# etri/bwa-mem-scale

Hardware: AMD Instinct MI355X
Metric: Mreads/sec through the GPU hot path (seed -> chain -> extend -> dedup, reads and index resident), 150bp SE vs a synthetic genome of GRCh38 size, at 1 MI355X; % HBM roofline in roofline.frac (higher is better)
Workload: dtype int64 intervals / int16 DP (two columns per register; int32 for queries beyond 191 bases or scores beyond 2^14)

## Files before the change

bwa-mem-scale_amd/csrc/api_extend.hip:

```cpp
#include <cstddef>

#include "stage_state.h"

using namespace bwams;

extern "C" {
static int ext_args(bwams_batch *b, StageState *s, const bwams_mem_opt_t *opt, ExtArgs *A) {
    const int64_t n1 = s->ch.nseq + 1;
    A->chains = s->ch.chains.p; A->n_chains = s->ch.n_chains; A->seeds = s->ch.seeds.p; A->n_seeds = s->ch.n_seeds;
    A->chain_off = s->ch.chain_off.as<int64_t>(); A->seed_off = s->ch.chain_off.as<int64_t>() + n1; A->enc = b->d_enc.p; A->cum = b->d_cum.p;
    A->nseq = s->ch.nseq; A->ref = b->idx->fmi.ref;
    int rc = dev_bns(b->idx, &A->bns);
    if (rc) return rc;
    A->opt = *opt; A->regs = s->ext.regs.p; A->srt = s->ext.srt.p; A->rmax = s->ext.rmax.as<int64_t>(); A->cnt = s->ext.cnt.as<int32_t>();
    A->ctr = b->d_ctr.p; A->state = s->ext.state.p; A->kreg = s->ext.kreg.p; A->cur = s->ext.cur.p; A->lim = s->ext.lim.p; A->sel_heavy = s->heavy.p;
    A->n_sel_heavy = &b->d_ctr.p->sel_heavy; A->sel_ticket = b->d_ctr.p->ext_sel_ticket; A->req_list = s->ext.req_list.p; A->rtask = nullptr;
    return BWAMS_OK;
}

static hipError_t ext_round_clear(bwams_batch *b) {
    DevCounters *c = b->d_ctr.p;
    return hipMemsetAsync(&c->ext_n_req, 0, (size_t)((char *)(c->ext_n_retry + 2) - (char *)&c->ext_n_req), b->stream);
}
static int ext_round_fetch(bwams_batch *b, int64_t *n_req, int64_t *n_rest, int64_t *n_l, int64_t *n_r) {
    DevCounters *h = b->h_ctr.p;
    BWAMS_HIP(hipMemcpyAsync(&h->ext_n_req, &b->d_ctr.p->ext_n_req, 3 * sizeof(unsigned long long), hipMemcpyDeviceToHost, b->stream));
    BWAMS_HIP(hipStreamSynchronize(b->stream));
    *n_req = (int64_t)h->ext_n_req; *n_rest = (int64_t)h->ext_n_rest;
    *n_l = (int64_t)(h->ext_n_tasks & 0xffffffffull); *n_r = (int64_t)(h->ext_n_tasks >> 32);
    return BWAMS_OK;
}

static int ext_plan(bwams_batch *b, StageState *s, const bwams_mem_opt_t *opt, int extend_all, ExtArgs *A) {
    const int64_t N1 = s->ch.n_seeds + 1, n1 = s->ch.nseq + 1;
    BWAMS_HIP(s->ext.regs.ensure_n((size_t)N1)); BWAMS_HIP(s->ext.srt.ensure_n((size_t)N1));
    BWAMS_HIP(s->ext.rmax.ensure((size_t)(s->ch.n_chains + 1) * 16)); BWAMS_HIP(s->ext.cnt.ensure((size_t)N1 * 6 * 4));
    BWAMS_HIP(s->ext.state.ensure_n((size_t)N1)); BWAMS_HIP(s->ext.kreg.ensure((size_t)N1 * 32)); BWAMS_HIP(s->ext.cur.ensure_n((size_t)n1));
    BWAMS_HIP(s->ext.lim.ensure_n((size_t)n1)); BWAMS_HIP(s->heavy.ensure_n((size_t)n1));
    BWAMS_HIP(s->ext.req_list.ensure_n((size_t)N1)); BWAMS_HIP(s->ext.rtask.ensure_n((size_t)N1));
    int rc = ext_args(b, s, opt, A);
    if (rc) return rc;
    BWAMS_HIP(hipMemsetAsync(&b->d_ctr.p->sel_heavy, 0, sizeof(unsigned long long), b->stream));
    BWAMS_HIP(ext_round_clear(b));
    launch_ext_heavy_list(*A, b->stream);
    BWAMS_HIP(hipMemsetAsync(s->ext.cur.p, 0, (size_t)n1 * 4, b->stream));
    BWAMS_HIP(hipMemsetAsync(s->ext.lim.p, 0, (size_t)n1 * 4, b->stream));
    launch_ext_plan(*A, extend_all, b->stream);
    return BWAMS_OK;
}

static int ext_build_flat(bwams_batch *b, StageState *s, const ExtArgs &A, const int32_t *list, int64_t n, int64_t tot[6]) {
    hipStream_t st = b->stream;
    const int64_t n1 = n + 1;
    BWAMS_HIP(s->ext.ewide.ensure((size_t)n1 * 6 * 8)); BWAMS_HIP(s->ext.eoffs.ensure((size_t)n1 * 6 * 8));
    launch_ext_widen(A, list, n, s->ext.ewide.as<int64_t>(), st);
    int rc = scan_rows(b, s->ext.ewide.as<int64_t>(), s->ext.eoffs.as<int64_t>(), 6, n1);
    if (rc) return rc;
    for (int r = 0; r < 6; ++r) BWAMS_HIP(hipMemcpyAsync(&tot[r], s->ext.eoffs.as<int64_t>() + r * n1 + n, 8, hipMemcpyDeviceToHost, st));
    BWAMS_HIP(hipStreamSynchronize(st));
    for (int r : {1, 2, 4, 5})
        if (tot[r] >= ((int64_t)1 << 31)) {
            set_last_error("extension task buffers exceed the 31-bit offsets of SeqPair; use smaller chunks");
            return BWAMS_ERR_CAPACITY;
        }
    s->ext.n_left = tot[0]; s->ext.lqer_b = tot[1]; s->ext.lref_b = tot[2];
    s->ext.n_right = tot[3]; s->ext.rqer_b = tot[4]; s->ext.rref_b = tot[5];
    BWAMS_HIP(s->ext.lpairs.ensure_n((size_t)(tot[0] + 1))); BWAMS_HIP(s->ext.rpairs.ensure_n((size_t)(tot[3] + 1)));
    const int64_t mx = tot[0] > tot[3] ? tot[0] : tot[3];
    BWAMS_HIP(s->ext.retry.ensure_n((size_t)(mx + 1)));
    s->ext.tasks_inplace = false;
    BWAMS_HIP(s->ext.lqer.ensure_n((size_t)tot[1] + 64)); BWAMS_HIP(s->ext.lref.ensure_n((size_t)tot[2] + 64));
    BWAMS_HIP(s->ext.rqer.ensure_n((size_t)tot[4] + 64)); BWAMS_HIP(s->ext.rref.ensure_n((size_t)tot[5] + 64));
    if (tot[0] + tot[3] > 0)
        launch_ext_build(A, list, n, s->ext.eoffs.as<int64_t>(), s->ext.lpairs.p, s->ext.lref.p, s->ext.lqer.p, s->ext.rpairs.p, s->ext.rref.p,
                         s->ext.rqer.p, nullptr, nullptr, st);
    return BWAMS_OK;
}

static int ext_build_round(bwams_batch *b, StageState *s, const ExtArgs &A, int64_t n_req, int64_t n_l, int64_t n_r, bool inplace) {
    if (!inplace) {
        int64_t tot[6] = {0, 0, 0, 0, 0, 0};
        if (int rc = ext_build_flat(b, s, A, A.req_list, n_req, tot)) return rc;
        if (tot[0] != n_l || tot[3] != n_r) {
            set_last_error("bwams_extend_run: the request list and its task counters disagree");
            return BWAMS_ERR_DEVICE;
        }
        return BWAMS_OK;
    }
    s->ext.n_left = n_l; s->ext.n_right = n_r;
    s->ext.lqer_b = s->ext.lref_b = s->ext.rqer_b = s->ext.rref_b = 0;
    BWAMS_HIP(s->ext.lpairs.ensure_n((size_t)(n_l + 1))); BWAMS_HIP(s->ext.rpairs.ensure_n((size_t)(n_r + 1)));
    const int64_t mx = n_l > n_r ? n_l : n_r;
    BWAMS_HIP(s->ext.retry.ensure_n((size_t)(mx + 1)));
    s->ext.tasks_inplace = true;
    BWAMS_HIP(s->ext.lsrc.ensure((size_t)(n_l + 1) * 16)); BWAMS_HIP(s->ext.rsrc.ensure((size_t)(n_r + 1) * 16));
    if (n_l + n_r > 0) launch_ext_build(A, A.req_list, n_req, nullptr, s->ext.lpairs.p, nullptr, nullptr, s->ext.rpairs.p,
                         nullptr, nullptr, s->ext.lsrc.as<int64_t>(), s->ext.rsrc.as<int64_t>(), b->stream);
    return BWAMS_OK;
}

int bwams_extend_build(bwams_batch_t *b, const bwams_mem_opt_t *opt, int64_t *n_left, int64_t *n_right) {
    if (!b || !b->stages || !b->stages->ch.done) {
        set_last_error("bwams_extend_build: run bwams_chain_run (or bwams_chain_upload) first");
        return BWAMS_ERR_ARG;
    }
    if (!b->idx->fmi.ref) {
        set_last_error("bwams_extend_build: the index was opened without its .0123 reference");
        return BWAMS_ERR_ARG;
    }
    int rc = check_opt(opt, "bwams_extend_build");
    if (rc) return rc;
    BWAMS_HIP(hipSetDevice(b->idx->device));
    StageState *s = b->stages;
    outdated(s, From::built);
    hipStream_t st = b->stream;
    ExtArgs A;
    BWAMS_HIP(hipEventRecord(s->ev[2], st));
    if ((rc = ext_plan(b, s, opt, 1, &A))) return rc;
    int64_t tot[6];
    if ((rc = ext_build_flat(b, s, A, nullptr, s->ch.n_seeds, tot))) return rc;
    BWAMS_HIP(hipEventRecord(s->ev[3], st));
    BWAMS_HIP(hipGetLastError());
    s->ext.built = true;
    s->opt = *opt;
    if (n_left) *n_left = tot[0];
    if (n_right) *n_right = tot[3];
    return BWAMS_OK;
}

static int run_side(bwams_batch *b, StageState *s, const ExtArgs &A, int right, int64_t *n_retry_out) {
    hipStream_t st = b->stream;
    bwams_seqpair_t *pairs = right ? s->ext.rpairs.p : s->ext.lpairs.p;
    const bool ip = s->ext.tasks_inplace;
    const uint8_t *ref = ip ? A.ref : (right ? s->ext.rref.p : s->ext.lref.p);
    const uint8_t *qer = ip ? A.enc : (right ? s->ext.rqer.p : s->ext.lqer.p);
    const int64_t *src = ip ? (right ? s->ext.rsrc.as<int64_t>() : s->ext.lsrc.as<int64_t>()) : nullptr;
    const int dir = ip && !right ? -1 : 1;
    const int64_t n = right ? s->ext.n_right : s->ext.n_left;
    SwParams prm;
    sw_params(A.opt, right ? A.opt.pen_clip3 : A.opt.pen_clip5, &prm);
    const int qmax = b->max_read_len > 1 ? b->max_read_len : 1;
    if (n == 0) return BWAMS_OK;
    unsigned long long *d_nretry = &b->d_ctr.p->ext_n_retry[right], *h_nretry = &b->h_ctr.p->ext_n_retry[right];
    bwams_seqpair_t *rp = A.rtask ? s->ext.rpairs.p : nullptr;
    if (bsw_list_bytes(n) > b->sw.d_bsw_list.cap) BWAMS_HIP(hipStreamSynchronize(st));
    BWAMS_HIP(b->sw.d_bsw_list.ensure(bsw_list_bytes(n), bsw_list_bytes(n + n / 4 + 1024)));
    if (int lrc = launch_bsw(pairs, n, ref, qer, A.opt.w, prm, qmax, b->d_ctr.p, b->cu_count, st, b->sw.d_bsw_list.p, s->aux, s->fork, s->join, src, dir)) {
        set_last_error(lrc == -2 ? "banded SW: a query longer than ~18000 bases does not fit the LDS kernel" : "banded SW: stream fork/join failed");
        return lrc == -2 ? BWAMS_ERR_UNSUPPORTED : BWAMS_ERR_DEVICE;
    }
    launch_ext_post(A, right, pairs, n, A.opt.w, 0, s->ext.retry.p, d_nretry, rp, st);
    BWAMS_HIP(hipMemcpyAsync(h_nretry, d_nretry, sizeof(unsigned long long), hipMemcpyDeviceToHost, st));
    BWAMS_HIP(hipStreamSynchronize(st));
    const unsigned long long nr = *h_nretry;
    if (nr) {
        if (launch_bsw(s->ext.retry.p, (int64_t)nr, ref, qer, A.opt.w << 1, prm, qmax, b->d_ctr.p, b->cu_count, st, b->sw.d_bsw_list.p, s->aux, s->fork, s->join, src, dir)) return BWAMS_ERR_DEVICE;
        launch_ext_post(A, right, s->ext.retry.p, (int64_t)nr, A.opt.w << 1, 1, nullptr, d_nretry, rp, st);
    }
    *n_retry_out += (int64_t)nr;
    return BWAMS_OK;
}

int bwams_extend_run(bwams_batch_t *b, const bwams_mem_opt_t *opt, int64_t *n_regs) {
    if (!b || !b->stages || !b->stages->ch.done) {
        set_last_error("bwams_extend_run: run bwams_chain_run (or bwams_chain_upload) first");
        return BWAMS_ERR_ARG;
    }
    if (!b->idx->fmi.ref) {
        set_last_error("bwams_extend_run: the index was opened without its .0123 reference");
        return BWAMS_ERR_ARG;
    }
    int rc = check_opt(opt, "bwams_extend_run");
    if (rc) return rc;
    int kMaxRounds = 6;
    if (knobs().ext_max_rounds > 0) kMaxRounds = knobs().ext_max_rounds;
    const bool adaptive_off = knobs().ext_all_rounds != 0;
    const bool inplace_on = knobs().ext_inplace != 0;
    StageState *s = b->stages;
    BWAMS_HIP(hipSetDevice(b->idx->device));
    hipStream_t st = b->stream;
    outdated(s, From::built);
    ExtArgs A;
    BWAMS_HIP(hipEventRecord(s->ev[10], st));
    BWAMS_HIP(hipMemsetAsync(&b->d_ctr.p->bsw_cells, 0, sizeof(unsigned long long), st));
    BWAMS_HIP(hipEventRecord(s->ev[2], st));
    if ((rc = ext_plan(b, s, opt, opt->extend_all != 0, &A))) return rc;
    A.rtask = s->ext.rtask.p;
    int64_t tot_left = 0, tot_right = 0;
    s->ext.n_retry_left = s->ext.n_retry_right = 0;
    int64_t n_req = 0, n_rest = 0, n_l = 0, n_r = 0;
    if ((rc = ext_round_fetch(b, &n_req, &n_rest, &n_l, &n_r))) return rc;
    int round = 0;
    for (;; ++round) {
        if ((rc = ext_build_round(b, s, A, n_req, n_l, n_r, inplace_on))) return rc;
        if (round == 0) { BWAMS_HIP(hipEventRecord(s->ev[3], st)); BWAMS_HIP(hipEventRecord(s->ev[4], st)); }
        tot_left += n_l; tot_right += n_r;
        if ((rc = run_side(b, s, A, 0, &s->ext.n_retry_left))) return rc;
        if (round == 0) { BWAMS_HIP(hipEventRecord(s->ev[5], st)); BWAMS_HIP(hipEventRecord(s->ev[6], st)); }
        if ((rc = run_side(b, s, A, 1, &s->ext.n_retry_right))) return rc;
        if (round == 0) { BWAMS_HIP(hipEventRecord(s->ev[7], st)); BWAMS_HIP(hipEventRecord(s->ev[8], st)); }
        BWAMS_HIP(ext_round_clear(b));
        const bool verbose_sel = knobs().verbose != 0;
        if (verbose_sel) BWAMS_HIP(hipMemsetAsync(b->d_ctr.p->dbg, 0, sizeof b->d_ctr.p->dbg, st));
        if (s->ch.n_seeds && launch_ext_select(A, b->cu_count, st, s->aux, s->fork, s->join)) {
            set_last_error("bwams_extend_run: stream fork/join failed");
            return BWAMS_ERR_DEVICE;
        }
        if (verbose_sel) {
            unsigned long long d[16];
            BWAMS_HIP(hipMemcpyAsync(d, b->d_ctr.p->dbg, sizeof d, hipMemcpyDeviceToHost, st));
            BWAMS_HIP(hipStreamSynchronize(st));
            if (d[0])
                fprintf(stderr, "[bwams_extend_run] selection walk, round %d: %llu reads, Mticks total %.2f fetch %.2f bulk scan %.2f ordered part %.2f (of it keep-anyway %.2f); "
                                "%llu slots, %llu keep-anyway calls; longest read: %.3f Mticks (fetch %.3f bulk %.3f ordered %.3f, of it keep-anyway %.3f), %llu slots "
                                "%llu calls, %llu kept regions\n",
                        round, d[0], d[1] / 1e6, d[2] / 1e6, d[3] / 1e6, d[4] / 1e6, d[5] / 1e6, d[6], d[7], d[8] / 1e6, d[9] / 1e6, d[10] / 1e6, d[11] / 1e6,
                        d[12] / 1e6, d[13], d[14], d[15]);
        }
        if (round == 0) BWAMS_HIP(hipEventRecord(s->ev[9], st));
        if ((rc = ext_round_fetch(b, &n_req, &n_rest, &n_l, &n_r))) return rc;
        if (n_req == 0) break;
        const bool few_left = !adaptive_off && (n_req + n_rest) * 32 < tot_left + tot_right;
        if (round + 1 >= kMaxRounds || few_left) {
            launch_ext_request_rest(A, st);
            if ((rc = ext_round_fetch(b, &n_req, &n_rest, &n_l, &n_r))) return rc;
        }
    }
    BWAMS_HIP(hipEventRecord(s->ev[11], st));
    BWAMS_HIP(hipGetLastError());
    s->ext.n_rounds = round + 1;
    s->ext.n_left = tot_left; s->ext.n_right = tot_right;
    s->ext.done = true;
    s->opt = *opt;
    if (n_regs) *n_regs = s->ch.n_seeds;
    return BWAMS_OK;
}

int bwams_extend_fetch(bwams_batch_t *b, bwams_alnreg_t *regs, int64_t reg_cap, int64_t *reg_off, int32_t *seed_aln) {
    if (!b || !b->stages || !(b->stages->ext.done || b->stages->ext.built)) {
        set_last_error("bwams_extend_fetch: no regions on the device");
        return BWAMS_ERR_ARG;
    }
    StageState *s = b->stages;
    if (s->ch.n_seeds > reg_cap) return BWAMS_ERR_CAPACITY;
    BWAMS_HIP(hipSetDevice(b->idx->device));
    hipStream_t st = b->stream;
    if (s->ch.n_seeds) BWAMS_HIP(hipMemcpyAsync(regs, s->ext.regs.p, (size_t)s->ch.n_seeds * sizeof(bwams_alnreg_t), hipMemcpyDeviceToHost, st));
    if (reg_off) BWAMS_HIP(hipMemcpyAsync(reg_off, s->ch.chain_off.as<int64_t>() + (s->ch.nseq + 1), (size_t)(s->ch.nseq + 1) * 8, hipMemcpyDeviceToHost, st));
    if (seed_aln && s->ch.n_seeds)
        BWAMS_HIP(hipMemcpy2DAsync(seed_aln, 4, reinterpret_cast<const char *>(s->ch.seeds.p) + offsetof(bwams_chain_seed_t, aln),
                                   sizeof(bwams_chain_seed_t), 4, (size_t)s->ch.n_seeds, hipMemcpyDeviceToHost, st));
    BWAMS_HIP(hipStreamSynchronize(st));
    return BWAMS_OK;
}

int bwams_extend_tasks_fetch(bwams_batch_t *b, int32_t side, bwams_seqpair_t *pairs, int64_t pair_cap, uint8_t *ref,
                             int64_t ref_cap, uint8_t *qer, int64_t qer_cap, int64_t *n_pairs, int64_t *ref_bytes,
                             int64_t *qer_bytes) {
    if (!b || !b->stages || !(b->stages->ext.built || b->stages->ext.done) || (side != 0 && side != 1)) {
        set_last_error("bwams_extend_tasks_fetch: no task lists on the device");
        return BWAMS_ERR_ARG;
    }
    if (b->stages->ext.tasks_inplace) {
        set_last_error("bwams_extend_tasks_fetch: bwams_extend_run extends in place and builds no flat task buffers; bwams_extend_build does");
        return BWAMS_ERR_ARG;
    }
    StageState *s = b->stages;
    const int64_t n = side ? s->ext.n_right : s->ext.n_left, rb = side ? s->ext.rref_b : s->ext.lref_b, qb = side ? s->ext.rqer_b : s->ext.lqer_b;
    if (n_pairs) *n_pairs = n;
    if (ref_bytes) *ref_bytes = rb;
    if (qer_bytes) *qer_bytes = qb;
    if (n > pair_cap || rb > ref_cap || qb > qer_cap) return BWAMS_ERR_CAPACITY;
    BWAMS_HIP(hipSetDevice(b->idx->device));
    hipStream_t st = b->stream;
    if (n) BWAMS_HIP(hipMemcpyAsync(pairs, side ? s->ext.rpairs.p : s->ext.lpairs.p, (size_t)n * sizeof(bwams_seqpair_t), hipMemcpyDeviceToHost, st));
    if (rb) BWAMS_HIP(hipMemcpyAsync(ref, side ? s->ext.rref.p : s->ext.lref.p, (size_t)rb, hipMemcpyDeviceToHost, st));
    if (qb) BWAMS_HIP(hipMemcpyAsync(qer, side ? s->ext.rqer.p : s->ext.lqer.p, (size_t)qb, hipMemcpyDeviceToHost, st));
    BWAMS_HIP(hipStreamSynchronize(st));
    return BWAMS_OK;
}
}
```

bwa-mem-scale_amd/csrc/bsw_extend.hip:

```cpp
#include "common.h"
#include "wave_ops.h"

namespace bwams {

namespace {

constexpr int kWavesPerBlock = 4;
constexpr int kTaskChunk = 8;
constexpr size_t kBswLdsMax = 160 * 1024;

__host__ __device__ __forceinline__ size_t bsw_row_bytes(int qmax) {
    return (((size_t)(qmax + 1) * 8 + (size_t)qmax + 64 + 15) / 16) * 16;
}

__device__ __forceinline__ int wave_incl_prefix_max(int v, int lane) {
#pragma unroll
    for (int o = 1; o < 64; o <<= 1) {
        const int t = __shfl_up(v, o);
        if (lane >= o) v = max(v, t);
    }
    return v;
}

__global__ __launch_bounds__(kWavesPerBlock * 64) void bsw_kernel(
// ... 390 lines not shown
                const int e = Ev[c];
                int h = Mv[c] > e ? Mv[c] : e;
                h = h > F ? h : F;
                int e2 = Mv[c] - oe_del;
                e2 = e2 > 0 ? e2 : 0;
                const int e1 = e - e_del;
                e2 = e2 > e1 ? e2 : e1;
                Hh[c] = h; E2[c] = e2;
            }
            const int h_in = grp_shr1<LPT>(Hh[kWin - 1], c_h, g);
#pragma unroll
            for (int c = 0; c < kWin; ++c) {
                const int j = jb + c;
                const bool act = in && j < end;
                const int hl = c ? Hh[c - 1] : h_in;
                if (act) {
                    const uint32_t he = (uint32_t)hl | ((uint32_t)E2[c] << 14);
                    row_eh[j] = (he & 0x0fffffffu) | (Qb[c] & ~0x0fffffffu);
                    const int k = (Hh[c] << 8) | j;
                    key = key > k ? key : k;
                    if (hl != 0 || E2[c] != 0) { first_nz = first_nz < j ? first_nz : j; last_nz = j; }
                }
            }
            {
                const int cl = end - 1 - jb;
                if (in && cl >= 0 && cl < kWin) {
                    int hv = Hh[0];
#pragma unroll
                    for (int c = 1; c < kWin; ++c) hv = cl == c ? Hh[c] : hv;
                    hlast = hv;
                }
            }
            if (wave_any(row && base + LPT * kWin < end)) {
                const int pm = grp_all_max<LPT>(scan);
                c_max = c_max > pm ? c_max : pm;
                c_h = grp_all_max<LPT>(g == LPT - 1 ? Hh[kWin - 1] : -1);
            }
        }
        key = grp_all_max<LPT>(key);
        first_nz = -grp_all_max<LPT>(-first_nz);
        last_nz = grp_all_max<LPT>(last_nz);
        hlast = grp_all_max<LPT>(hlast);
        const int m = row ? key >> 8 : 0, mj = row ? key & 0xff : -1;
        const int h1f = row ? hlast : h1;
        if (alive) {
            if (g == 0) {
                row_eh[end] = (uint32_t)h1f | (row_eh[end] & 0xf0000000u);
            }
            if (row) cells += (unsigned long long)(g == 0 ? end - beg : 0);
            const int j_exit = row ? end : beg;
            if (j_exit == qlen) {
                max_ie = gscore > h1f ? max_ie : i;
                gscore = gscore > h1f ? gscore : h1f;
            }
            bool fin = m == 0;
            if (!fin) {
                if (m > mx) {
                    mx = m; max_i = i; max_j = mj;
                    int d = mj - i;
                    d = d < 0 ? -d : d;
                    max_off = max_off > d ? max_off : d;
                } else if (prm.zdrop > 0) {
                    if (i - max_i > mj - max_j) fin = mx - m - ((i - max_i) - (mj - max_j)) * e_del > prm.zdrop;
                    else fin = mx - m - ((mj - max_j) - (i - max_i)) * e_ins > prm.zdrop;
                }
            }
            if (!fin) {
                const int nbeg = first_nz < end ? first_nz : end;
                int jj;
                if (h1f != 0) jj = end;
                else if (last_nz >= nbeg) jj = last_nz;
                else jj = nbeg - 1;
                beg = nbeg;
                end = jj + 2 < qlen ? jj + 2 : qlen;
                ++i;
                fin = i >= tlen;
            }
            if (fin) {
                if (g == 0) {
                    bwams_seqpair_t *o = &pairs[cur];
                    o->score = mx; o->qle = max_j + 1; o->tle = max_i + 1; o->gtle = max_ie + 1; o->gscore = gscore; o->max_off = max_off;
                }
                alive = false;
            }
        }
    }
    for (int o = 32; o > 0; o >>= 1) cells += ((unsigned long long)__shfl_down((unsigned)(cells >> 32), o) << 32) | (unsigned)__shfl_down((unsigned)cells, o);
    if (lane == 0 && cells) atomicAdd(&ctr->bsw_cells, cells);
}


namespace pk {
__device__ __forceinline__ uint32_t add(uint32_t a, uint32_t b) { uint32_t d; asm("v_pk_add_u16 %0, %1, %2" : "=v"(d) : "v"(a), "v"(b)); return d; }
__device__ __forceinline__ uint32_t sub(uint32_t a, uint32_t b) { uint32_t d; asm("v_pk_sub_i16 %0, %1, %2" : "=v"(d) : "v"(a), "v"(b)); return d; }
__device__ __forceinline__ uint32_t max(uint32_t a, uint32_t b) { uint32_t d; asm("v_pk_max_i16 %0, %1, %2" : "=v"(d) : "v"(a), "v"(b)); return d; }
__device__ __forceinline__ uint32_t max0(uint32_t a) { uint32_t d; asm("v_pk_max_i16 %0, %1, 0" : "=v"(d) : "v"(a)); return d; }
__device__ __forceinline__ uint32_t minu(uint32_t a, uint32_t b) { uint32_t d; asm("v_pk_min_u16 %0, %1, %2" : "=v"(d) : "v"(a), "v"(b)); return d; }
__device__ __forceinline__ uint32_t mul(uint32_t a, uint32_t b) { uint32_t d; asm("v_pk_mul_lo_u16 %0, %1, %2" : "=v"(d) : "v"(a), "v"(b)); return d; }
__device__ __forceinline__ uint32_t hi2(uint32_t a) { return __builtin_amdgcn_perm(a, a, 0x03020302u); }
__device__ __forceinline__ uint32_t lo2(uint32_t a) { return __builtin_amdgcn_perm(a, a, 0x01000100u); }
__device__ __forceinline__ uint32_t bfi(uint32_t mask, uint32_t a, uint32_t b) { return (a & mask) | (b & ~mask); }
template <int CTRL> __device__ __forceinline__ int qdpp(int v) { return __builtin_amdgcn_update_dpp(0, v, CTRL, 0xF, 0xF, false); }
__device__ __forceinline__ int quad_all_max(int v) {
    int t = qdpp<0xB1>(v);
    v = v > t ? v : t;
    t = qdpp<0x4E>(v);
    return v > t ? v : t;
}
}

constexpr int kPkNeg = -16384;
#ifndef BWAMS_PK_WAVES
#define BWAMS_PK_WAVES 2
#endif
constexpr int kPkWaves = BWAMS_PK_WAVES;

__host__ __device__ __forceinline__ bool bsw_pk_eligible(const SwParams &prm) {
    for (int i = 0; i < 5; ++i)
        if (prm.mat[i * 5 + 4] != -1 || prm.mat[4 * 5 + i] != -1) return false;
    return prm.e_ins >= 0 && prm.e_ins <= 64 && prm.e_del >= 0 && prm.e_del <= 64 && prm.o_ins >= 0 && prm.o_ins + prm.e_ins < 8000 &&
           prm.o_del >= 0 && prm.o_del + prm.e_del < 8000;
}

__global__ __launch_bounds__(kPkWaves * 64) void bsw_pk_kernel(
    bwams_seqpair_t *__restrict__ pairs, const int32_t *__restrict__ list, const unsigned long long *n_list_p,
    const uint8_t *__restrict__ ref, const uint8_t *__restrict__ qer, int w0, SwParams prm, DevCounters *ctr, unsigned long long *head,
    int cols, const int64_t *__restrict__ src, int dir) {
    extern __shared__ __align__(16) uint32_t pk_lds[];
    constexpr int LPT = 4, TPW = 16;
    const int lane = threadIdx.x & 63, g = lane & (LPT - 1), q = lane / LPT;
    const int P = cols >> 1;
    uint32_t *const t_hp = pk_lds + 16 + (size_t)((threadIdx.x >> 6) * TPW + q) * (size_t)((5 * P) / 2 + 6);
    uint32_t *const t_ep = t_hp + P + 2;
    uint16_t *const t_sel = reinterpret_cast<uint16_t *>(t_ep + P + 2);
    uint16_t *const t_hp16 = reinterpret_cast<uint16_t *>(t_hp), *const t_ep16 = reinterpret_cast<uint16_t *>(t_ep);
    const int o_del = prm.o_del, e_del = prm.e_del, o_ins = prm.o_ins, e_ins = prm.e_ins;
    const int oe_del = o_del + e_del, oe_ins = o_ins + e_ins;
    uint2 *const pk_tab16 = reinterpret_cast<uint2 *>(pk_lds);
    if (threadIdx.x < 5) {
        const int t = threadIdx.x;
        pk_tab16[t] = make_uint2((uint32_t)(uint16_t)(int16_t)prm.mat[t * 5 + 0] | ((uint32_t)(uint16_t)(int16_t)prm.mat[t * 5 + 1] << 16),
                                 (uint32_t)(uint16_t)(int16_t)prm.mat[t * 5 + 2] | ((uint32_t)(uint16_t)(int16_t)prm.mat[t * 5 + 3] << 16));
    }
    __syncthreads();
    const uint32_t ONE = 0x00010001u, TWO = 0x00020002u, C257 = 0x01010101u;
    const uint32_t OEI = (uint32_t)oe_ins * 0x10001u, OED = (uint32_t)oe_del * 0x10001u, EDX = (uint32_t)e_del * 0x10001u;
    const uint32_t E1X = (uint32_t)e_ins * 0x10001u, E2X = (uint32_t)(2 * e_ins) * 0x10001u;
    const uint32_t NEGP = (uint32_t)(uint16_t)(int16_t)kPkNeg * 0x10001u;
    const int64_t n_list = (int64_t)*n_list_p;
    const unsigned long long kLeaders = 0x1111111111111111ull;
    int64_t pid = 0, pid_end = 0;
    bool exhausted = false;
    bool alive = false;
    int cur = 0, qlen = 0, tlen = 0, h0 = 0, w = 0, i = 0, beg = 0, end = 0;
    int mx = 0, max_i = -1, max_j = -1, max_ie = -1, gscore = -1, max_off = 0, tb_next = 4;
    const uint8_t *tr = ref;
    unsigned long long cells = 0;
    bool start_row = true, row = false;
    int base = 0, h1 = 0, key = -1, hlast = -1, c_max = kPkNeg, c_h = 0;
    uint32_t nzl = 0u, nzf = 0u;
    uint2 tt = make_uint2(0u, 0u);

    for (;;) {
        const unsigned long long need_m = __ballot(!alive);
        if (need_m) {
            if (pid >= pid_end && !exhausted) {
                pid = (int64_t)wave_ticket(head, (unsigned long long)kQuadChunk);
                pid_end = pid + kQuadChunk < n_list ? pid + kQuadChunk : n_list;
                if (pid >= n_list) { exhausted = true; pid_end = pid; }
            }
            const int avail = (int)(pid_end - pid);
            const int nq = __popcll(need_m & kLeaders);
            const int rank = __popcll(need_m & kLeaders & ((1ull << (q * LPT)) - 1ull));
            if (!alive && rank < avail) {
                cur = list[pid + rank];
                const bwams_seqpair_t sp = pairs[cur];
                qlen = sp.len2; tlen = sp.len1; h0 = sp.h0;
                const uint8_t *tq = qer + (src ? src[2 * (int64_t)sp.id] : (int64_t)sp.idq);
                tr = ref + (src ? src[2 * (int64_t)sp.id + 1] : (int64_t)sp.idr);
                start_row = true;
                for (int p = g; p <= (qlen >> 1); p += LPT) {
                    uint32_t hh = 0, ss = 0;
#pragma unroll
                    for (int k = 0; k < 2; ++k) {
                        const int c = 2 * p + k;
                        int h = 0;
                        if (c <= qlen) { h = h0; if (c >= 1) { h = h0 - oe_ins - (c - 1) * e_ins; h = h > 0 ? h : 0; } }
                        uint32_t qb = c < qlen ? (uint32_t)tq[c * dir] : 4u;
                        const uint32_t sel = qb < 4u ? 2u * qb : 0x0du;
                        hh |= (uint32_t)h << (16 * k);
                        ss |= sel << (8 * k);
                    }
                    t_hp[p] = hh; t_ep[p] = 0u; t_sel[p] = (uint16_t)ss;
                }
                w = w0;
                {
                    int max_ins = (int)((double)(qlen * prm.max_sc + prm.end_bonus - o_ins) / e_ins + 1.);
                    max_ins = max_ins > 1 ? max_ins : 1;
                    w = w < max_ins ? w : max_ins;
                    int max_del = (int)((double)(qlen * prm.max_sc + prm.end_bonus - o_del) / e_del + 1.);
                    max_del = max_del > 1 ? max_del : 1;
                    w = w < max_del ? w : max_del;
                }
                mx = h0; max_i = -1; max_j = -1; max_ie = -1; gscore = -1; max_off = 0;
                beg = 0; end = qlen; i = 0;
                alive = tlen > 0;
                if (!alive && g == 0) {
                    bwams_seqpair_t *o = &pairs[cur];
                    o->score = mx; o->qle = 0; o->tle = 0; o->gtle = 0; o->gscore = -1; o->max_off = 0;
                }
                tb_next = alive ? (int)tr[0] : 4;
            }
            pid += nq < avail ? nq : avail;
            if (exhausted && !wave_any(alive)) break;
        }

        if (alive && start_row) {
            int tb = tb_next;
            tb = tb > 4 ? 4 : tb;
            if (i + 1 < tlen) tb_next = tr[(i + 1) * dir];
            tt = pk_tab16[tb];
            if (beg < i - w) beg = i - w;
            if (end > i + w + 1) end = i + w + 1;
            if (end > qlen) end = qlen;
            h1 = 0;
            if (beg == 0) {
                h1 = h0 - (o_del + e_del * (i + 1));
                h1 = h1 < 0 ? 0 : h1;
            }
            row = beg < end;
            key = -1; hlast = -1; nzl = 0u; nzf = 0u;
            c_max = kPkNeg; c_h = 0;
            base = beg & ~3;
            start_row = false;
        }
        {
            const bool in = alive && row;
            const int jb = base + g * 8;
            const bool inr = in && jb < cols;
            int lo = beg - jb, hi = end - jb;
            lo = lo < 0 ? 0 : (lo > 8 ? 8 : lo);
            hi = hi < 0 ? 0 : (hi > 8 ? 8 : hi);
            const uint32_t m8 = inr ? ((1u << hi) - 1u) & ~((1u << lo) - 1u) : 0u;
            const int pj = inr ? (jb >> 1) : 0;
            const uint2 hpa = *reinterpret_cast<const uint2 *>(t_hp + pj), hpb = *reinterpret_cast<const uint2 *>(t_hp + pj + 2);
            const uint2 epa = *reinterpret_cast<const uint2 *>(t_ep + pj), epb = *reinterpret_cast<const uint2 *>(t_ep + pj + 2);
            uint2 sl2;
            sl2.x = *reinterpret_cast<const uint32_t *>(t_sel + pj);
            sl2.y = *reinterpret_cast<const uint32_t *>(t_sel + pj + 2);
            const uint32_t hpv[4] = {hpa.x, hpa.y, hpb.x, hpb.y}, epv[4] = {epa.x, epa.y, epb.x, epb.y};
            const uint32_t slv[4] = {__builtin_amdgcn_perm(sl2.x, sl2.x, 0x01010000u) + 0x01000100u, __builtin_amdgcn_perm(sl2.x, sl2.x, 0x03030202u) + 0x01000100u,
                                     __builtin_amdgcn_perm(sl2.y, sl2.y, 0x01010000u) + 0x01000100u, __builtin_amdgcn_perm(sl2.y, sl2.y, 0x03030202u) + 0x01000100u};
            uint32_t AM[4], M[4], E[4], PX[4], JE[4], JP[4];
            JE[0] = (uint32_t)(jb * e_ins) * 0x10001u + ((uint32_t)e_ins << 16);
            JP[0] = (uint32_t)jb * 0x10001u + 0x00020001u;
#pragma unroll
            for (int c = 1; c < 4; ++c) { JE[c] = pk::add(JE[c - 1], E2X); JP[c] = pk::add(JP[c - 1], TWO); }
            uint32_t Hm[4], T1[4], T2[4];
#pragma unroll
            for (int c = 0; c < 4; ++c) {
                const uint32_t blo = (uint32_t)__builtin_amdgcn_sbfe((int)m8, 2 * c, 1), bhi = (uint32_t)__builtin_amdgcn_sbfe((int)m8, 2 * c + 1, 1);
                AM[c] = pk::bfi(0xffffu, blo, bhi);
            }
#pragma unroll
            for (int c = 0; c < 4; ++c) { Hm[c] = hpv[c] & AM[c]; E[c] = epv[c] & AM[c]; }
#pragma unroll
            for (int c = 0; c < 4; ++c) T1[c] = pk::add(Hm[c], __builtin_amdgcn_perm(tt.y, tt.x, slv[c]));
#pragma unroll
            for (int c = 0; c < 4; ++c) T2[c] = pk::minu(Hm[c], ONE);
#pragma unroll
            for (int c = 0; c < 4; ++c) M[c] = pk::mul(T1[c], T2[c]);
#pragma unroll
            for (int c = 0; c < 4; ++c) T1[c] = pk::sub(M[c], OEI);
#pragma unroll
            for (int c = 0; c < 4; ++c) T1[c] = pk::max0(T1[c]);
#pragma unroll
            for (int c = 0; c < 4; ++c) T1[c] = pk::add(T1[c], JE[c]);
#pragma unroll
            for (int c = 0; c < 4; ++c) PX[c] = pk::max(T1[c], T1[c] << 16);
#pragma unroll
            for (int c = 1; c < 4; ++c) PX[c] = pk::max(PX[c], pk::hi2(PX[c - 1]));
            int scan = (int)(PX[3] >> 16);
            {
                int t = pk::qdpp<0x90>(scan);
                scan = scan > t ? scan : t;
                t = pk::qdpp<0x44>(scan);
                scan = scan > t ? scan : t;
            }
            int Lex = pk::qdpp<0x90>(scan);
            Lex = g == 0 ? kPkNeg : Lex;
            Lex = Lex > c_max ? Lex : c_max;
            const uint32_t Lexp = pk::lo2((uint32_t)Lex);
            uint32_t Hn[4], E2[4], F4[4], ME[4];
#pragma unroll
            for (int c = 0; c < 4; ++c) F4[c] = __builtin_amdgcn_alignbit(PX[c], c ? PX[c - 1] : NEGP, 16);
#pragma unroll
            for (int c = 0; c < 4; ++c) { F4[c] = pk::max(F4[c], Lexp); E2[c] = pk::sub(M[c], OED); }
#pragma unroll
            for (int c = 0; c < 4; ++c) { F4[c] = pk::sub(F4[c], JE[c]); T1[c] = pk::sub(E[c], EDX); ME[c] = pk::max(M[c], E[c]); }
#pragma unroll
            for (int c = 0; c < 4; ++c) { F4[c] = pk::add(F4[c], E1X); E2[c] = pk::max(E2[c], T1[c]); }
#pragma unroll
            for (int c = 0; c < 4; ++c) { F4[c] = pk::max0(F4[c]); E2[c] = pk::max0(E2[c]); }
#pragma unroll
            for (int c = 0; c < 4; ++c) Hn[c] = pk::max(ME[c], F4[c]);
            const int h3 = (int)(Hn[3] >> 16);
            int hin = pk::qdpp<0x90>(h3);
            hin = g == 0 ? c_h : hin;
            uint32_t HL[4];
            HL[0] = __builtin_amdgcn_alignbit(Hn[0], (uint32_t)hin << 16, 16);
#pragma unroll
            for (int c = 1; c < 4; ++c) HL[c] = __builtin_amdgcn_alignbit(Hn[c], Hn[c - 1], 16);
            if (m8) {
                *reinterpret_cast<uint2 *>(t_hp + pj) = make_uint2(pk::bfi(AM[0], HL[0], hpv[0]), pk::bfi(AM[1], HL[1], hpv[1]));
                *reinterpret_cast<uint2 *>(t_hp + pj + 2) = make_uint2(pk::bfi(AM[2], HL[2], hpv[2]), pk::bfi(AM[3], HL[3], hpv[3]));
                *reinterpret_cast<uint2 *>(t_ep + pj) = make_uint2(pk::bfi(AM[0], E2[0], epv[0]), pk::bfi(AM[1], E2[1], epv[1]));
                *reinterpret_cast<uint2 *>(t_ep + pj + 2) = make_uint2(pk::bfi(AM[2], E2[2], epv[2]), pk::bfi(AM[3], E2[3], epv[3]));
            }
            int lkey = -1;
#pragma unroll
            for (int c = 0; c < 4; ++c) {
                const uint32_t ha = Hn[c] & AM[c];
                const int k0 = (int)__builtin_amdgcn_perm(ha, JP[c], 0x0c050400u), k1 = (int)__builtin_amdgcn_perm(ha, JP[c], 0x0c070602u);
                const int kk = k0 > k1 ? k0 : k1;
                lkey = lkey > kk ? lkey : kk;
            }
            {
                uint32_t NF[4], NA[4], NB[4];
#pragma unroll
                for (int c = 0; c < 4; ++c) NF[c] = (HL[c] | E2[c]) & AM[c];
#pragma unroll
                for (int c = 0; c < 4; ++c) { NF[c] = pk::minu(NF[c], ONE); NB[c] = pk::sub(C257, JP[c]); }
#pragma unroll
                for (int c = 0; c < 4; ++c) { NA[c] = pk::mul(NF[c], JP[c]); NB[c] = pk::mul(NF[c], NB[c]); }
                NA[0] = pk::max(NA[0], NA[1]); NA[2] = pk::max(NA[2], NA[3]); NB[0] = pk::max(NB[0], NB[1]); NB[2] = pk::max(NB[2], NB[3]);
                NA[0] = pk::max(NA[0], NA[2]); NB[0] = pk::max(NB[0], NB[2]);
                nzl = pk::max(nzl, NA[0]);
                nzf = pk::max(nzf, NB[0]);
            }
            lkey = m8 ? lkey : -1;
            key = key > lkey ? key : lkey;
            {
                const int oe = hi - 1;
                if (m8 && jb + hi == end) {
                    uint32_t hv = Hn[0];
                    hv = (oe >> 1) == 1 ? Hn[1] : hv;
                    hv = (oe >> 1) == 2 ? Hn[2] : hv;
                    hv = (oe >> 1) == 3 ? Hn[3] : hv;
                    hlast = (int)((hv >> ((oe & 1) << 4)) & 0xffffu);
                }
            }
            if (in && base == (beg & ~3) && h1 != 0 && g == 0) t_hp16[beg] = (uint16_t)h1;
            const int pm = pk::qdpp<0xFF>(scan);
            const int ch = pk::qdpp<0xFF>(h3);
            const bool more = in && base + LPT * 8 < end;
            if (more) {
                c_max = c_max > pm ? c_max : pm;
                c_h = ch;
                base += LPT * 8;
            }
            const int rkey = pk::quad_all_max(key), rhl = pk::quad_all_max(hlast);
            const int a_ = (int)(nzl & 0xffffu), b_ = (int)(nzl >> 16), c_ = (int)(nzf & 0xffffu), d_ = (int)(nzf >> 16);
            int last_nz = pk::quad_all_max(a_ > b_ ? a_ : b_) - 1;
            int first_nz = 256 - pk::quad_all_max(c_ > d_ ? c_ : d_);
            if (alive && !more) {
                if (row && h1 != 0) {
                    first_nz = first_nz < beg ? first_nz : beg;
                    last_nz = last_nz > beg ? last_nz : beg;
                }
                const int m = row ? rkey >> 8 : 0, mj = row ? (rkey & 0xff) - 1 : -1;
                const int h1f = row ? rhl : h1;
                if (g == 0) { t_hp16[end] = (uint16_t)h1f; t_ep16[end] = 0; }
                if (row) cells += (unsigned long long)(g == 0 ? end - beg : 0);
                const int j_exit = row ? end : beg;
                if (j_exit == qlen) {
                    max_ie = gscore > h1f ? max_ie : i;
                    gscore = gscore > h1f ? gscore : h1f;
                }
                bool fin = m == 0;
                if (!fin) {
                    if (m > mx) {
                        mx = m; max_i = i; max_j = mj;
                        int d = mj - i;
                        d = d < 0 ? -d : d;
                        max_off = max_off > d ? max_off : d;
                    } else if (prm.zdrop > 0) {
                        if (i - max_i > mj - max_j) fin = mx - m - ((i - max_i) - (mj - max_j)) * e_del > prm.zdrop;
                        else fin = mx - m - ((mj - max_j) - (i - max_i)) * e_ins > prm.zdrop;
                    }
                }
                if (!fin) {
                    const int nbeg = first_nz < end ? first_nz : end;
                    int jj;
                    if (h1f != 0) jj = end;
                    else if (last_nz >= nbeg) jj = last_nz;
                    else jj = nbeg - 1;
                    beg = nbeg;
                    end = jj + 2 < qlen ? jj + 2 : qlen;
                    ++i;
                    fin = i >= tlen;
                }
                if (fin) {
                    if (g == 0) {
                        bwams_seqpair_t *o = &pairs[cur];
                        o->score = mx; o->qle = max_j + 1; o->tle = max_i + 1; o->gtle = max_ie + 1; o->gscore = gscore; o->max_off = max_off;
                    }
                    alive = false;
                }
                start_row = true;
            }
        }
    }
    for (int o = 32; o > 0; o >>= 1) cells += ((unsigned long long)__shfl_down((unsigned)(cells >> 32), o) << 32) | (unsigned)__shfl_down((unsigned)cells, o);
    if (lane == 0 && cells) atomicAdd(&ctr->bsw_cells, cells);
}

__global__ void bsw_reset_kernel(DevCounters *ctr) {
    for (int i = 0; i < 4; ++i) ctr->bsw_head[i] = 0;
    for (int i = 0; i < kNumBswClass; ++i) ctr->bsw_cls_cnt[i] = ctr->bsw_cls_head[i] = 0;
}

}

int launch_bsw(bwams_seqpair_t *pairs, int64_t n, const uint8_t *ref, const uint8_t *qer, int w, const SwParams &prm, int qmax,
               DevCounters *ctr, int cu_count, hipStream_t st, int32_t *list, hipStream_t *aux, hipEvent_t fork, hipEvent_t *join,
               const int64_t *src, int dir) {
    bsw_reset_kernel<<<1, 1, 0, st>>>(ctr);
    if (n <= 0) return 0;
    bsw_classify_kernel<<<(unsigned)((n + 1023) / 1024), 1024, 0, st>>>(pairs, n, prm.max_sc, list, ctr->bsw_cls_cnt);
    int64_t blocks = (n + kWavesPerBlock - 1) / kWavesPerBlock;
    const int64_t maxb = (int64_t)cu_count * 8;
    if (blocks > maxb) blocks = maxb;
    hipStream_t q[5] = {st, st, st, st, st};
    const int n_aux = aux ? 4 : 0;
    if (n_aux) {
        if (hipEventRecord(fork, st) != hipSuccess) return -1;
        for (int c = 0; c < n_aux; ++c) {
            q[c + 1] = aux[c];
            if (hipStreamWaitEvent(q[c + 1], fork, 0) != hipSuccess) return -1;
        }
    }
    const unsigned B = (unsigned)blocks, T = kWavesPerBlock * 64;
    unsigned long long *cnt = ctr->bsw_cls_cnt, *hd = ctr->bsw_cls_head;
    auto pk_lds = [](int cols) { return (size_t)64 + (size_t)kPkWaves * 16 * ((size_t)(cols / 2) * 10 + 24); };
    {
        static std::mutex mu;
        static bool done[64] = {};
        int dev = 0;
        if (hipGetDevice(&dev) != hipSuccess) return -1;
        std::lock_guard<std::mutex> g(mu);
        if (dev < 0 || dev >= 64 || !done[dev]) {
            if (hipFuncSetAttribute(reinterpret_cast<const void *>(bsw_qwin_kernel<kBswLpt, kBswWin>), hipFuncAttributeMaxDynamicSharedMemorySize,
                                    (int)((size_t)kWavesPerBlock * (64 / kBswLpt) * 192 * 4)) != hipSuccess) return -1;
            if (hipFuncSetAttribute(reinterpret_cast<const void *>(bsw_pk_kernel), hipFuncAttributeMaxDynamicSharedMemorySize, (int)pk_lds(192)) != hipSuccess) return -1;
            if (dev >= 0 && dev < 64) done[dev] = true;
        }
    }
    const bool pk_env = knobs().bsw_pk != 0;
    if (pk_env && bsw_pk_eligible(prm)) {
        static const int kCols[5] = {32, 64, 96, 144, 192};
        const unsigned Bp = (unsigned)((int64_t)B * kWavesPerBlock / kPkWaves);
        for (int c = 4; c >= 0; --c)
            bsw_pk_kernel<<<Bp, kPkWaves * 64, pk_lds(kCols[c]), q[c]>>>(pairs, list + (int64_t)c * n, cnt + c, ref, qer, w, prm, ctr, hd + c, kCols[c], src, dir);
    } else {
    bsw_qwin_kernel<kBswLpt, kBswWin><<<B, T, (size_t)kWavesPerBlock * (64 / kBswLpt) * 192 * 4, q[4]>>>(pairs, list + 4 * n, cnt + 4, ref, qer, w, prm, ctr, hd + 4, 192, src, dir);
    bsw_qwin_kernel<kBswLpt, kBswWin><<<B, T, (size_t)kWavesPerBlock * (64 / kBswLpt) * 144 * 4, q[3]>>>(pairs, list + 3 * n, cnt + 3, ref, qer, w, prm, ctr, hd + 3, 144, src, dir);
    bsw_qwin_kernel<kBswLpt, kBswWin><<<B, T, (size_t)kWavesPerBlock * (64 / kBswLpt) * 96 * 4, q[2]>>>(pairs, list + 2 * n, cnt + 2, ref, qer, w, prm, ctr, hd + 2, 96, src, dir);
    bsw_qwin_kernel<kBswLpt, kBswWin><<<B, T, (size_t)kWavesPerBlock * (64 / kBswLpt) * 64 * 4, q[1]>>>(pairs, list + 1 * n, cnt + 1, ref, qer, w, prm, ctr, hd + 1, 64, src, dir);
    bsw_qwin_kernel<kBswLpt, kBswWin><<<B, T, (size_t)kWavesPerBlock * (64 / kBswLpt) * 32 * 4, q[0]>>>(pairs, list + 0 * n, cnt + 0, ref, qer, w, prm, ctr, hd + 0, 32, src, dir);
    }
    {
        const int waves = bsw_lds_waves(qmax);
        if (waves < 1) return -2;
        const size_t lds = bsw_row_bytes(qmax) * (size_t)waves;
        if (lds > 48 * 1024)
            (void)hipFuncSetAttribute(reinterpret_cast<const void *>(bsw_kernel),
                                      hipFuncAttributeMaxDynamicSharedMemorySize, (int)lds);
        int64_t lblocks = (n + waves - 1) / waves;
        const int64_t lcap = qmax > 16 * kQuadCpl[4] - 1 ? maxb : (int64_t)cu_count * 2;
        if (lblocks > lcap) lblocks = lcap;
        bsw_kernel<<<(unsigned)lblocks, waves * 64, lds, q[0]>>>(pairs, n, ref, qer, w, prm, qmax, -1, ctr, &ctr->bsw_head[3], list + 5 * n, cnt + 5, src, dir);
    }
    if (n_aux)
        for (int c = 0; c < n_aux; ++c) {
            if (hipEventRecord(join[c], q[c + 1]) != hipSuccess) return -1;
            if (hipStreamWaitEvent(st, join[c], 0) != hipSuccess) return -1;
        }
    return 0;
}
size_t bsw_list_bytes(int64_t n) { return (size_t)kNumBswClass * (size_t)(n > 0 ? n : 1) * sizeof(int32_t); }

int bsw_lds_waves(int qmax) {
    const size_t waves = kBswLdsMax / bsw_row_bytes(qmax);
    return waves < (size_t)kWavesPerBlock ? (int)waves : kWavesPerBlock;
}

}
```

Baseline: 10.01.

## Prefetch task metadata per chunk and cooperatively fill query rows across whole wave

When a wave grabs a chunk of tasks, each of the first kQuadChunk lanes loads one task's pair record, offsets, first ref base and band width, and these are broadcast by shuffle to the lanes that take a task. Query-profile and initial H-row setup is then done by all 64 lanes together, one task at a time, using 4-byte vector loads instead of a per-quad strided loop. The aim is to cut the serialized refill cost in the banded SW packed kernel. It adds shuffles, a per-slot fill loop and LDS fences, plus optional timing instrumentation behind a debug macro and a verbose flag.

```diff
diff --git a/bwa-mem-scale_amd/csrc/api_extend.hip b/bwa-mem-scale_amd/csrc/api_extend.hip
--- a/bwa-mem-scale_amd/csrc/api_extend.hip
+++ b/bwa-mem-scale_amd/csrc/api_extend.hip
@@ -145,6 +145,8 @@
     bwams_seqpair_t *rp = A.rtask ? s->ext.rpairs.p : nullptr;
     if (bsw_list_bytes(n) > b->sw.d_bsw_list.cap) BWAMS_HIP(hipStreamSynchronize(st));
     BWAMS_HIP(b->sw.d_bsw_list.ensure(bsw_list_bytes(n), bsw_list_bytes(n + n / 4 + 1024)));
+    const bool verbose_bsw = knobs().verbose != 0;
+    if (verbose_bsw) BWAMS_HIP(hipMemsetAsync(b->d_ctr.p->dbg + 40, 0, 8 * sizeof(unsigned long long), st));
     if (int lrc = launch_bsw(pairs, n, ref, qer, A.opt.w, prm, qmax, b->d_ctr.p, b->cu_count, st, b->sw.d_bsw_list.p, s->aux, s->fork, s->join, src, dir)) {
         set_last_error(lrc == -2 ? "banded SW: a query longer than ~18000 bases does not fit the LDS kernel" : "banded SW: stream fork/join failed");
         return lrc == -2 ? BWAMS_ERR_UNSUPPORTED : BWAMS_ERR_DEVICE;
@@ -152,6 +154,14 @@
     launch_ext_post(A, right, pairs, n, A.opt.w, 0, s->ext.retry.p, d_nretry, rp, st);
     BWAMS_HIP(hipMemcpyAsync(h_nretry, d_nretry, sizeof(unsigned long long), hipMemcpyDeviceToHost, st));
     BWAMS_HIP(hipStreamSynchronize(st));
+    if (verbose_bsw) {
+        unsigned long long d[8];
+        BWAMS_HIP(hipMemcpy(d, b->d_ctr.p->dbg + 40, sizeof d, hipMemcpyDeviceToHost));
+        if (d[6])
+            fprintf(stderr, "[run_side] bsw_pk_kernel, %s, %lld tasks: %llu waves, Mticks of wave-time %.2f, in the refill branch %.2f (%.1f %%), in the pass %.2f; "
+                            "%llu refill events, %llu slots filled, %llu iterations\n",
+                    right ? "right" : "left", (long long)n, d[6], d[0] / 1e6, d[1] / 1e6, 100. * (double)d[1] / (double)d[0], d[2] / 1e6, d[3], d[4], d[5]);
+    }
     const unsigned long long nr = *h_nretry;
     if (nr) {
         if (launch_bsw(s->ext.retry.p, (int64_t)nr, ref, qer, A.opt.w << 1, prm, qmax, b->d_ctr.p, b->cu_count, st, b->sw.d_bsw_list.p, s->aux, s->fork, s->join, src, dir)) return BWAMS_ERR_DEVICE;
diff --git a/bwa-mem-scale_amd/csrc/bsw_extend.hip b/bwa-mem-scale_amd/csrc/bsw_extend.hip
--- a/bwa-mem-scale_amd/csrc/bsw_extend.hip
+++ b/bwa-mem-scale_amd/csrc/bsw_extend.hip
@@ -566,6 +566,9 @@
     int64_t pid = 0, pid_end = 0;
     bool exhausted = false;
     bool alive = false;
+    int64_t pid0 = 0, s_qo = 0, s_to = 0;
+    int s_cur = 0, s_tlen = 0, s_w = 0;
+    uint32_t s_qh = 0u;
     int cur = 0, qlen = 0, tlen = 0, h0 = 0, w = 0, i = 0, beg = 0, end = 0;
     int mx = 0, max_i = -1, max_j = -1, max_ie = -1, gscore = -1, max_off = 0, tb_next = 4;
     const uint8_t *tr = ref;
@@ -574,60 +577,115 @@
     int base = 0, h1 = 0, key = -1, hlast = -1, c_max = kPkNeg, c_h = 0;
     uint32_t nzl = 0u, nzf = 0u;
     uint2 tt = make_uint2(0u, 0u);
+#ifdef BWAMS_BSWDBG
+    const unsigned long long T0 = __builtin_amdgcn_s_memtime();
+    unsigned long long t_refill = 0, t_pass = 0, n_events = 0, n_filled = 0, n_iter = 0;
+#endif
 
     for (;;) {
         const unsigned long long need_m = __ballot(!alive);
         if (need_m) {
+#ifdef BWAMS_BSWDBG
+            const unsigned long long Ta = __builtin_amdgcn_s_memtime();
+#endif
             if (pid >= pid_end && !exhausted) {
                 pid = (int64_t)wave_ticket(head, (unsigned long long)kQuadChunk);
                 pid_end = pid + kQuadChunk < n_list ? pid + kQuadChunk : n_list;
                 if (pid >= n_list) { exhausted = true; pid_end = pid; }
+                pid0 = pid;
+                if (lane < kQuadChunk && pid + lane < pid_end) {
+                    s_cur = list[pid + lane];
+                    const bwams_seqpair_t *sp = &pairs[s_cur];
+                    const int l2 = sp->len2, hh0 = sp->h0;
+                    s_tlen = sp->len1;
+                    if (src) { const int64_t id = sp->id; s_qo = src[2 * id]; s_to = src[2 * id + 1]; }
+                    else { s_qo = (int64_t)sp->idq; s_to = (int64_t)sp->idr; }
+                    uint32_t tb = s_tlen > 0 ? (uint32_t)ref[s_to] : 4u;
+                    tb = tb > 4u ? 4u : tb;
+                    s_qh = (uint32_t)l2 | ((uint32_t)hh0 << 8) | (tb << 24);
+                    int ww = w0;
+                    int max_ins = (int)((double)(l2 * prm.max_sc + prm.end_bonus - o_ins) / e_ins + 1.);
+                    max_ins = max_ins > 1 ? max_ins : 1;
+                    ww = ww < max_ins ? ww : max_ins;
+                    int max_del = (int)((double)(l2 * prm.max_sc + prm.end_bonus - o_del) / e_del + 1.);
+                    max_del = max_del > 1 ? max_del : 1;
+                    s_w = ww < max_del ? ww : max_del;
+                }
             }
             const int avail = (int)(pid_end - pid);
             const int nq = __popcll(need_m & kLeaders);
             const int rank = __popcll(need_m & kLeaders & ((1ull << (q * LPT)) - 1ull));
-            if (!alive && rank < avail) {
-                cur = list[pid + rank];
-                const bwams_seqpair_t sp = pairs[cur];
-                qlen = sp.len2; tlen = sp.len1; h0 = sp.h0;
-                const uint8_t *tq = qer + (src ? src[2 * (int64_t)sp.id] : (int64_t)sp.idq);
-                tr = ref + (src ? src[2 * (int64_t)sp.id + 1] : (int64_t)sp.idr);
-                start_row = true;
-                for (int p = g; p <= (qlen >> 1); p += LPT) {
-                    uint32_t hh = 0, ss = 0;
-#pragma unroll
+            if (avail > 0) {
+                const bool take = !alive && rank < avail;
+                const int sk = take ? (int)(pid - pid0) + rank : 0;
+                const int f_cur = __shfl(s_cur, sk), f_tlen = __shfl(s_tlen, sk), f_w = __shfl(s_w, sk);
+                const uint32_t f_qh = (uint32_t)__shfl((int)s_qh, sk);
+                const int64_t f_qo = shfl64(s_qo, sk), f_to = shfl64(s_to, sk);
+                if (take) {
+                    cur = f_cur; qlen = (int)(f_qh & 0xffu); h0 = (int)((f_qh >> 8) & 0x3fffu); tlen = f_tlen; w = f_w;
+                    tr = ref + f_to;
+                    start_row = true;
+                    mx = h0; max_i = -1; max_j = -1; max_ie = -1; gscore = -1; max_off = 0;
+                    beg = 0; end = qlen; i = 0;
+                    alive = tlen > 0;
+                    if (!alive && g == 0) {
+                        bwams_seqpair_t *o = &pairs[cur];
+                        o->score = mx; o->qle = 0; o->tle = 0; o->gtle = 0; o->gscore = -1; o->max_off = 0;
+                    }
+                    tb_next = (int)(f_qh >> 24);
+                }
+                for (unsigned long long fill_m = __ballot(take) & kLeaders; fill_m; fill_m &= fill_m - 1ull) {
+                    const int sl = __ffsll((long long)fill_m) - 1;
+                    const int f_qlen = __builtin_amdgcn_readlane(qlen, sl), f_h0 = __builtin_amdgcn_readlane(h0, sl);
+                    const uint8_t *const f_q = qer + readlane64(f_qo, sl);
+                    uint32_t *const f_hp = pk_lds + 16 + (size_t)((threadIdx.x >> 6) * TPW + (sl >> 2)) * (size_t)((5 * P) / 2 + 6);
+                    uint32_t *const f_ep = f_hp + P + 2;
+                    uint16_t *const f_sel = reinterpret_cast<uint16_t *>(f_ep + P + 2);
+                    const int c0 = 4 * lane, p_last = f_qlen >> 1;
+                    const bool full = c0 + 3 < f_qlen, edge = !full && c0 < f_qlen;
+                    uint32_t v = 0u, b0 = 4u, b1 = 4u, b2 = 4u;
+                    if (full) __builtin_memcpy(&v, dir > 0 ? f_q + c0 : f_q - c0 - 3, 4);
+                    if (edge) {
+                        const int last = f_qlen - 1;
+                        b0 = f_q[c0 * dir];
+                        b1 = f_q[(c0 + 1 < last ? c0 + 1 : last) * dir];
+                        b2 = f_q[(c0 + 2 < last ? c0 + 2 : last) * dir];
+                    }
+                    b1 = c0 + 1 < f_qlen ? b1 : 4u;
+                    b2 = c0 + 2 < f_qlen ? b2 : 4u;
+                    const uint32_t qw = full ? (dir > 0 ? v : __builtin_amdgcn_perm(v, v, 0x00010203u)) : (b0 | (b1 << 8) | (b2 << 16) | 0x04000000u);
+                    uint32_t hh[2] = {0u, 0u}, ss[2] = {0u, 0u};
+    #pragma unroll
+                    for (int k = 0; k < 4; ++k) {
+                        const int c = c0 + k;
+                        int h = 0;
+                        if (c <= f_qlen) { h = f_h0; if (c >= 1) { h = f_h0 - oe_ins - (c - 1) * e_ins; h = h > 0 ? h : 0; } }
+                        const uint32_t qb = (qw >> (8 * k)) & 0xffu;
+                        const uint32_t sel = qb < 4u ? 2u * qb : 0x0du;
+                        hh[k >> 1] |= (uint32_t)h << (16 * (k & 1));
+                        ss[k >> 1] |= sel << (8 * (k & 1));
+                    }
+    #pragma unroll
                     for (int k = 0; k < 2; ++k) {
-                        const int c = 2 * p + k;
-                        int h = 0;
-                        if (c <= qlen) { h = h0; if (c >= 1) { h = h0 - oe_ins - (c - 1) * e_ins; h = h > 0 ? h : 0; } }
-                        uint32_t qb = c < qlen ? (uint32_t)tq[c * dir] : 4u;
-                        const uint32_t sel = qb < 4u ? 2u * qb : 0x0du;
-                        hh |= (uint32_t)h << (16 * k);
-                        ss |= sel << (8 * k);
+                        const int p = 2 * lane + k;
+                        if (p <= p_last) { f_hp[p] = hh[k]; f_ep[p] = 0u; f_sel[p] = (uint16_t)ss[k]; }
                     }
-                    t_hp[p] = hh; t_ep[p] = 0u; t_sel[p] = (uint16_t)ss;
-                }
-                w = w0;
-                {
-                    int max_ins = (int)((double)(qlen * prm.max_sc + prm.end_bonus - o_ins) / e_ins + 1.);
-                    max_ins = max_ins > 1 ? max_ins : 1;
-                    w = w < max_ins ? w : max_ins;
-                    int max_del = (int)((double)(qlen * prm.max_sc + prm.end_bonus - o_del) / e_del + 1.);
-                    max_del = max_del > 1 ? max_del : 1;
-                    w = w < max_del ? w : max_del;
-                }
-                mx = h0; max_i = -1; max_j = -1; max_ie = -1; gscore = -1; max_off = 0;
-                beg = 0; end = qlen; i = 0;
-                alive = tlen > 0;
-                if (!alive && g == 0) {
-                    bwams_seqpair_t *o = &pairs[cur];
-                    o->score = mx; o->qle = 0; o->tle = 0; o->gtle = 0; o->gscore = -1; o->max_off = 0;
-                }
-                tb_next = alive ? (int)tr[0] : 4;
+                }
+                __builtin_amdgcn_fence(__ATOMIC_RELEASE, "wavefront");
+                asm volatile("s_waitcnt lgkmcnt(0)" ::: "memory");
+                __builtin_amdgcn_fence(__ATOMIC_ACQUIRE, "wavefront");
             }
             pid += nq < avail ? nq : avail;
+#ifdef BWAMS_BSWDBG
+            asm volatile("s_waitcnt vmcnt(0) lgkmcnt(0)" ::: "memory");
+            t_refill += __builtin_amdgcn_s_memtime() - Ta;
+            ++n_events; n_filled += (unsigned long long)(nq < avail ? nq : avail);
+#endif
             if (exhausted && !wave_any(alive)) break;
         }
+#ifdef BWAMS_BSWDBG
+        const unsigned long long Tb = __builtin_amdgcn_s_memtime();
+#endif
 
         if (alive && start_row) {
             int tb = tb_next;
@@ -824,7 +882,19 @@
                 start_row = true;
             }
         }
-    }
+#ifdef BWAMS_BSWDBG
+        asm volatile("s_waitcnt vmcnt(0) lgkmcnt(0)" ::: "memory");
+        t_pass += __builtin_amdgcn_s_memtime() - Tb;
+        ++n_iter;
+#endif
+    }
+#ifdef BWAMS_BSWDBG
+    if (lane == 0) {
+        unsigned long long *d = ctr->dbg + 40;
+        atomicAdd(&d[0], __builtin_amdgcn_s_memtime() - T0); atomicAdd(&d[1], t_refill); atomicAdd(&d[2], t_pass);
+        atomicAdd(&d[3], n_events); atomicAdd(&d[4], n_filled); atomicAdd(&d[5], n_iter); atomicAdd(&d[6], 1ull);
+    }
+#endif
     for (int o = 32; o > 0; o >>= 1) cells += ((unsigned long long)__shfl_down((unsigned)(cells >> 32), o) << 32) | (unsigned)__shfl_down((unsigned)cells, o);
     if (lane == 0 && cells) atomicAdd(&ctr->bsw_cells, cells);
 }
```

Result: faster. 10.36, median of 6 (+3.5%).
